# haoheliu/AudioLDM2

Hardware: AMD Instinct MI355X
Metric: audio_seconds_per_second (higher is better)
Workload: dtype f32 storage/accumulate; each product = 6 bf16 MFMA partial products of exact 3-part operand splits (fp32-grade); 1 GPU; audioldm2-full: batch 8 prompts/GPU x 1 GPU, 10.24 s @16 kHz, 200 DDIM steps, CFG 3.5, eta 1.0, n_candidates 1; one step = sample_log + VAE decode + HiFi-GAN + D2H of the waveform; synthetic conditioning, random-init weights, host-CPU RNG noise; global_batch=8, parallelism=prompt-sharded replicas x1, weight_broadcast_bytes=0

## Files before the change

audioldm2_amd/csrc/api.hip:

```cpp
#include "common.h"
#include <string.h>

namespace aldm {
static thread_local char g_err[512] = "";
void set_error(const char* fmt, ...) {
    va_list ap;
    va_start(ap, fmt);
    vsnprintf(g_err, sizeof(g_err), fmt, ap);
    va_end(ap);
}
}

extern "C" int aldm_version(void) { return 26; }
extern "C" const char* aldm_last_error(void) { return aldm::g_err; }
```

audioldm2_amd/csrc/norm.hip:

```cpp
#include <stdlib.h>
#include "igemm_epilogue.h"

namespace aldm {

constexpr int GN_ITERS = 16;
constexpr int GN_UNROLL = 8;

struct GnPart {
    float n, mean, m2;
};

__device__ __forceinline__ void gn_merge(double& n, double& mean, double& m2, double nb, double mb, double m2b) {
    if (nb <= 0.0) return;
    const double nt = n + nb;
    const double dlt = mb - mean;
    mean += dlt * (nb / nt);
    m2 += m2b + dlt * dlt * (n * nb / nt);
    n = nt;
}

template <bool FUSED>
__global__ __launch_bounds__(256) void gn_partial_kernel(const float* __restrict__ x1,
                                                         const float* __restrict__ x2, int P,
                                                         int C1, int C2, int G, int cols, int rows,
                                                         int chunk_px, float* __restrict__ ws, float eps,
                                                         const float* __restrict__ gamma,
                                                         const float* __restrict__ beta,
                                                         float* __restrict__ scale, float* __restrict__ shift, int gpb,
                                                         char* __restrict__ dst = nullptr, char* __restrict__ dst_raw = nullptr,
                                                         int parts = 3, int act = ALDM_ACT_NONE, int raw_parts = 3,
                                                         float f16_scale = 0.f) {
    const int C = C1 + C2;
    const int Cg4 = (C / G) >> 2;
    const int b = blockIdx.y;
    const int chunk = FUSED ? 0 : blockIdx.x;
    const int g_lo = FUSED ? blockIdx.x * gpb : 0;
    const int c4_lo = g_lo * Cg4, C4 = c4_lo + gpb * Cg4;
    const int p0 = chunk * chunk_px;
    const int p1 = min(P, p0 + chunk_px);
    const int tid = threadIdx.x;
    const int tx = tid % cols, ty = tid / cols;
    __shared__ GnPart ps[256];
    const int npass = (C4 - c4_lo + cols - 1) / cols;
    __shared__ double gacc[64][3];
    if (tid < 64) gacc[tid][0] = gacc[tid][1] = gacc[tid][2] = 0.0;
    __syncthreads();
    for (int cp = 0; cp < npass; ++cp) {
        const int c4 = c4_lo + cp * cols + tx;
        GnPart part = {0.f, 0.f, 0.f};
        if (ty < rows && c4 < C4 && p0 + ty < p1) {
            const int c = c4 << 2;
            const bool first = c < C1;
            const float* src = first ? x1 + (int64_t)b * P * C1 + c : x2 + (int64_t)b * P * C2 + (c - C1);
            const int pitch = first ? C1 : C2;
            float sa[GN_UNROLL], sq[GN_UNROLL];
#pragma unroll
            for (int u = 0; u < GN_UNROLL; ++u) sa[u] = sq[u] = 0.f;
            int p = p0 + ty;
            const f32x4 pv = *reinterpret_cast<const f32x4*>(src + (int64_t)p * pitch);
            const float pivot = fmaxf(fminf(pv[0], pv[1]), fminf(fmaxf(pv[0], pv[1]), pv[2]));
            int cnt = 0;
            for (; p + (GN_UNROLL - 1) * rows < p1; p += GN_UNROLL * rows) {
                f32x4 v[GN_UNROLL];
#pragma unroll
                for (int u = 0; u < GN_UNROLL; ++u)
                    v[u] = *reinterpret_cast<const f32x4*>(src + (int64_t)(p + u * rows) * pitch) - pivot;
#pragma unroll
                for (int u = 0; u < GN_UNROLL; ++u) {
// ... 87 lines not shown
            scale[(int64_t)b * C + c] = sc;
            shift[(int64_t)b * C + c] = sh;
            if (dst) {
                lsc[c - g_lo * Cg] = sc;
                lsh[c - g_lo * Cg] = sh;
            }
        }
        if (dst) {
            __syncthreads();
            const int c_lo = g_lo * Cg, sw = (gpb * Cg) >> 3;
            for (int i = tid; i < P * sw; i += 256) {
                const int p = i / sw;
                const int cl = (i - p * sw) << 3;
                const int c = c_lo + cl;
                const int64_t row = (int64_t)b * P + p;
                const float* src = c < C1 ? x1 + row * C1 + c : x2 + row * C2 + (c - C1);
                f32x4 v0 = *reinterpret_cast<const f32x4*>(src);
                f32x4 v1 = *reinterpret_cast<const f32x4*>(src + 4);
                const int64_t off = (row * (C >> 5) + (c >> 5)) * (64 * parts) + (c & 31) * 2;
                u32x2 p0[3], p1[3];
                if (dst_raw) {
                    const int64_t roff = (row * (C >> 5) + (c >> 5)) * (64 * raw_parts) + (c & 31) * 2;
                    split4_parts(v0, p0, raw_parts);
                    split4_parts(v1, p1, raw_parts);
#pragma unroll
                    for (int q = 0; q < 3; ++q)
                        if (q < raw_parts)
                            *reinterpret_cast<u32x4*>(dst_raw + roff + q * 64) = u32x4{p0[q][0], p0[q][1], p1[q][0], p1[q][1]};
                }
#pragma unroll
                for (int e = 0; e < 4; ++e) {
// ... 7 lines not shown
                        v1[e] = silu_fast(v1[e]);
                    }
                }
                split4_fmt(v0, p0, parts, f16_scale);
                split4_fmt(v1, p1, parts, f16_scale);
#pragma unroll
                for (int q = 0; q < 3; ++q)
                    if (q < parts) *reinterpret_cast<u32x4*>(dst + off + q * 64) = u32x4{p0[q][0], p0[q][1], p1[q][0], p1[q][1]};
            }
        }
    } else if (tid < G) {
        double* w = reinterpret_cast<double*>(ws) + ((int64_t)(b * gridDim.x + chunk) * G + tid) * 3;
        w[0] = gacc[tid][0];
        w[1] = gacc[tid][1];
        w[2] = gacc[tid][2];
    }
}

__global__ __launch_bounds__(256) void gn_finalize_kernel(const float* __restrict__ ws, int chunks,
                                                          int P, int C, int G, float eps,
                                                          const float* __restrict__ gamma,
                                                          const float* __restrict__ beta,
                                                          float* __restrict__ scale,
                                                          float* __restrict__ shift) {
    const int b = blockIdx.x;
    __shared__ float s_mean[64], s_rstd[64];
    __shared__ double s_part[256][3];
    const int Cg = C / G;
    const double* wsd = reinterpret_cast<const double*>(ws);
    const int LPG = 256 / G >= 1 ? 256 / G : 1;
    {
        const int g = threadIdx.x / LPG, l = threadIdx.x % LPG;
        double n = 0.0, mean = 0.0, m2 = 0.0;
        if (g < G) {
            for (int ch = l; ch < chunks; ch += LPG) {
                const double* w = wsd + ((int64_t)(b * chunks + ch) * G + g) * 3;
                gn_merge(n, mean, m2, w[0], w[1], w[2]);
            }
        }
        s_part[threadIdx.x][0] = n;
        s_part[threadIdx.x][1] = mean;
        s_part[threadIdx.x][2] = m2;
    }
    __syncthreads();
    if (threadIdx.x < G) {
        const int g = threadIdx.x;
        double n = 0.0, mean = 0.0, m2 = 0.0;
        for (int l = 0; l < LPG; ++l) gn_merge(n, mean, m2, s_part[g * LPG + l][0], s_part[g * LPG + l][1], s_part[g * LPG + l][2]);
        double var = n > 0.0 ? m2 / n : 0.0;
        if (var < 0.0) var = 0.0;
        s_mean[g] = (float)mean;
        s_rstd[g] = (float)(1.0 / sqrt(var + (double)eps));
    }
    __syncthreads();
    for (int c = threadIdx.x; c < C; c += blockDim.x) {
        const int g = c / Cg;
        const float ga = gamma ? gamma[c] : 1.f;
        const float be = beta ? beta[c] : 0.f;
        const float sc = s_rstd[g] * ga;
        scale[(int64_t)b * C + c] = sc;
        shift[(int64_t)b * C + c] = be - s_mean[g] * sc;
    }
}

constexpr int LN_MAXV = 8;

template <int MAXV, int R, bool RMS = false>
__global__ __launch_bounds__(256) void layernorm_kernel(const float* __restrict__ x,
                                                        float* __restrict__ y, int M, int C,
                                                        const float* __restrict__ gamma,
                                                        const float* __restrict__ beta, float eps,
                                                        void* __restrict__ y_split, int parts, float f16_scale) {
    const int lane = threadIdx.x & 63;
    const int row0 = (blockIdx.x * 4 + (threadIdx.x >> 6)) * R;
    if (row0 >= M) return;
    const int C4 = C >> 2;
// ... 152 lines not shown
        pl.cols = c4b < 256 ? c4b : 256;
        pl.rows = 256 / pl.cols;
        pl.chunk_px = P;
        pl.chunks = 1;
        pl.passes = (c4b + pl.cols - 1) / pl.cols;
    } else {
        pl.form = ALDM_GN_CHUNKED;
        gn_geometry(P, C, &pl.cols, &pl.rows, &pl.chunk_px, &pl.chunks);
        pl.passes = (C / 4 + pl.cols - 1) / pl.cols;
    }
    const int px = P < pl.chunk_px ? P : pl.chunk_px;
    pl.active = pl.cols * (pl.rows < px ? pl.rows : px);
    return pl;
}

}

using namespace aldm;

extern "C" int64_t aldm_gn_ws_floats(int B, int P, int C, int G) {
    int cols, rows, chunk_px, chunks;
    gn_geometry(P, C, &cols, &rows, &chunk_px, &chunks);
    return (int64_t)B * chunks * G * 6 + 2;
}

extern "C" int aldm_split_rows(const float* x1, const float* x2, int C1, int C2, int64_t rows, int P, const float* scale,
                               const float* shift, int act, void* dst, void* dst_raw, int parts, void* stream);
extern "C" int aldm_split_rows_f16(const float* x1, const float* x2, int C1, int C2, int64_t rows, int P, const float* scale,
                                   const float* shift, int act, float slope, void* dst, void* dst_raw, int raw_parts, float f16_scale,
                                   void* stream);
// ... 8 lines not shown
    ALDM_CHECK(!want_split || (C % 32 == 0 && C1 % 8 == 0 && C2 % 8 == 0),
               "aldm_groupnorm_plan: a split image needs (C1+C2) %% 32 == 0, C1 %% 8 == 0 (C1=%d C2=%d)", C1, C2);
    const GnPlan pl = groupnorm_plan(B, P, C, C1, G, want_split != 0);
    if (form) *form = pl.form;
    if (group_slices) *group_slices = pl.gs;
    if (groups_per_block) *groups_per_block = pl.gpb;
    if (chunks) *chunks = pl.chunks;
    if (chunk_px) *chunk_px = pl.chunk_px;
    if (cols) *cols = pl.cols;
    if (rows) *rows = pl.rows;
    if (passes) *passes = pl.passes;
    if (active_threads) *active_threads = pl.active;
    return 0;
}

static int groupnorm_launch(const float* x1, const float* x2, int B, int P, int C1, int C2, int G, float eps,
                            const float* gamma, const float* beta, float* scale, float* shift, float* ws, void* dst,
                            void* dst_raw, int parts, int act, void* stream, int raw_parts = 0, float f16_scale = 0.f) {
    if (raw_parts == 0) raw_parts = parts;
    if (!x2) C2 = 0;
    const int C = C1 + C2;
    ALDM_CHECK(x1 && scale && shift && ws, "aldm_groupnorm_stats: null pointer");
    ws = reinterpret_cast<float*>((reinterpret_cast<uintptr_t>(ws) + 7) & ~uintptr_t(7));
    ALDM_CHECK(G > 0 && G <= 64 && C % G == 0 && (C / G) % 4 == 0 && C1 % 4 == 0,
               "aldm_groupnorm_stats: need C%%G==0, (C/G)%%4==0, C1%%4==0 (C1=%d C2=%d G=%d)", C1, C2, G);
    const GnPlan pl = groupnorm_plan(B, P, C, C1, G, dst != nullptr);
    hipStream_t st = (hipStream_t)stream;
    if (pl.form == ALDM_GN_FUSED_SPLIT) {
        hipLaunchKernelGGL(gn_partial_kernel<true>, dim3(pl.gs, B), dim3(256), 0, st, x1, x2, P, C1, C2, G, pl.cols, pl.rows, P, ws,
                           eps, gamma, beta, scale, shift, pl.gpb, reinterpret_cast<char*>(dst),
                           reinterpret_cast<char*>(dst_raw), parts, act, raw_parts, f16_scale);
        ALDM_LAUNCH_CHECK("aldm_groupnorm_split");
        return 0;
    }
    if (pl.form == ALDM_GN_FUSED) {
        hipLaunchKernelGGL(gn_partial_kernel<true>, dim3(pl.gs, B), dim3(256), 0, st, x1, x2, P, C1, C2, G, pl.cols,
                           pl.rows, P, ws, eps, gamma, beta, scale, shift, pl.gpb, nullptr, nullptr, 3, ALDM_ACT_NONE);
    } else {
        hipLaunchKernelGGL(gn_partial_kernel<false>, dim3(pl.chunks, B), dim3(256), 0, st, x1, x2, P, C1, C2, G,
                           pl.cols, pl.rows, pl.chunk_px, ws, eps, gamma, beta, scale, shift, G);
        hipLaunchKernelGGL(gn_finalize_kernel, dim3(B), dim3(256), 0, st, ws, pl.chunks, P, C, G, eps, gamma,
                           beta, scale, shift);
    }
    ALDM_LAUNCH_CHECK("aldm_groupnorm_stats");
    if (dst) {
        if (f16_scale != 0.f)
            return aldm_split_rows_f16(x1, x2, C1, C2, (int64_t)B * P, P, scale, shift, act, 0.f, dst, dst_raw, raw_parts, f16_scale, stream);
        return aldm_split_rows(x1, x2, C1, C2, (int64_t)B * P, P, scale, shift, act, dst, dst_raw, parts, stream);
    }
    return 0;
}

extern "C" int aldm_groupnorm_stats(const float* x1, const float* x2, int B, int P, int C1, int C2,
                                    int G, float eps, const float* gamma, const float* beta,
                                    float* scale, float* shift, float* ws, void* stream) {
    return groupnorm_launch(x1, x2, B, P, C1, C2, G, eps, gamma, beta, scale, shift, ws, nullptr, nullptr, 3, ALDM_ACT_NONE,
                            stream);
}

extern "C" int aldm_groupnorm_split(const float* x1, const float* x2, int B, int P, int C1, int C2, int G, float eps,
                                    const float* gamma, const float* beta, int act, float* scale, float* shift, float* ws,
                                    void* dst, void* dst_raw, int parts, void* stream) {
    if (!x2) C2 = 0;
    ALDM_CHECK(dst != nullptr && (parts == 2 || parts == 3) && (C1 + C2) % 32 == 0 && C1 % 8 == 0 && C2 % 8 == 0,
               "aldm_groupnorm_split: need dst, parts 2|3, (C1+C2) %% 32 == 0, C1 %% 8 == 0 (C1=%d C2=%d)", C1, C2);
    ALDM_CHECK(act == ALDM_ACT_NONE || act == ALDM_ACT_SILU, "aldm_groupnorm_split: activation %d not supported", act);
    ALDM_CHECK(((reinterpret_cast<uintptr_t>(dst) | reinterpret_cast<uintptr_t>(dst_raw)) & 15) == 0,
               "aldm_groupnorm_split: split images must be 16-byte aligned");
    return groupnorm_launch(x1, x2, B, P, C1, C2, G, eps, gamma, beta, scale, shift, ws, dst, dst_raw, parts, act, stream);
}

extern "C" int aldm_groupnorm_split_f16(const float* x1, const float* x2, int B, int P, int C1, int C2, int G, float eps,
                                        const float* gamma, const float* beta, int act, float* scale, float* shift, float* ws,
                                        void* dst, void* dst_raw, int raw_parts, float f16_scale, void* stream) {
    if (!x2) C2 = 0;
    ALDM_CHECK(dst != nullptr && f16_scale > 0.0f && (raw_parts == 2 || raw_parts == 3) && (C1 + C2) % 32 == 0 && C1 % 8 == 0 && C2 % 8 == 0,
               "aldm_groupnorm_split_f16: need dst, f16_scale > 0, raw_parts 2|3, (C1+C2) %% 32 == 0, C1 %% 8 == 0 (C1=%d C2=%d)", C1, C2);
    ALDM_CHECK(act == ALDM_ACT_NONE || act == ALDM_ACT_SILU, "aldm_groupnorm_split_f16: activation %d not supported", act);
    ALDM_CHECK(((reinterpret_cast<uintptr_t>(dst) | reinterpret_cast<uintptr_t>(dst_raw)) & 15) == 0,
               "aldm_groupnorm_split_f16: split images must be 16-byte aligned");
    return groupnorm_launch(x1, x2, B, P, C1, C2, G, eps, gamma, beta, scale, shift, ws, dst, dst_raw, 2, act, stream, raw_parts, f16_scale);
}

static int layernorm_launch(const float* x, float* y, void* y_split, int parts, int M, int C, const float* gamma,
                            const float* beta, float eps, void* stream, const char* name, bool rms = false, float f16_scale = 0.f) {
    ALDM_CHECK(parts == 2 || parts == 3, "%s: parts must be 2 or 3", name);
    ALDM_CHECK(x && (y || y_split) && gamma && (beta || rms), "%s: null pointer", name);
    ALDM_CHECK(C % 4 == 0 && C <= 256 * LN_MAXV, "%s: C=%d must be a multiple of 4 and <= %d", name, C, 256 * LN_MAXV);
    ALDM_CHECK(y_split == nullptr || (C % 32 == 0 && (reinterpret_cast<uintptr_t>(y_split) & 15) == 0),
               "%s: a split-image output needs C %% 32 == 0 and 16-byte alignment", name);
    hipStream_t st = (hipStream_t)stream;
#define ALDM_LN(V_, R_)                                                                                             \
    do {                                                                                                            \
        if (rms)                                                                                                    \
            hipLaunchKernelGGL((layernorm_kernel<V_, R_, true>), dim3(cdiv(M, 4 * R_)), dim3(256), 0, st, x, y, M, C, \
                               gamma, beta, eps, y_split, parts, f16_scale);                                        \
// ... 80 lines not shown
```

audioldm2_amd/lib.py:

```python
from __future__ import annotations

import ctypes as C
import os

_HERE = os.path.dirname(os.path.abspath(__file__))
LIB_PATH = os.environ.get("ALDM_LIB_PATH") or os.path.join(_HERE, "libaldm_hip.so")
ABI_VERSION = 26

ACT_NONE, ACT_SILU, ACT_LRELU, ACT_TANH, ACT_LOGCLAMP, ACT_GELU, ACT_GELU_TANH = range(7)
B_PACKED, B_NT = 0, 1
EPI_PLAIN, EPI_GEGLU, EPI_QKV = 0, 1, 2
GN_CHUNKED, GN_FUSED, GN_FUSED_SPLIT = 0, 1, 2
FMT_BF16, FMT_F16 = 0, 1
EPI_FORM_GENERIC, EPI_FORM_PLAIN, EPI_FORM_ROWBIAS, EPI_FORM_RES = range(4)


class IgemmDesc(C.Structure):

    _fields_ = [
        ("x1", C.c_void_p), ("x2", C.c_void_p),
        ("C1", C.c_int32), ("C2", C.c_int32),
        ("pix1", C.c_int32), ("pix2", C.c_int32),
        ("B", C.c_int32), ("H", C.c_int32), ("W", C.c_int32),
        ("up_h", C.c_int32), ("up_w", C.c_int32),
# ... 76 lines not shown
    "aldm_igemm_mma": (C.c_int, [C.c_int]),
    "aldm_split_bytes": (C.c_int64, [C.c_int, C.c_int]),
    "aldm_pack_split_bf16": (C.c_int, [C.c_void_p, C.c_void_p, C.c_int, C.c_int, C.c_void_p]),
    "aldm_pack_weight": (C.c_int, [C.c_void_p, C.c_void_p, C.c_int, C.c_int, C.c_int, C.c_int,
                                   C.c_int, C.c_int, C.c_int, C.c_void_p]),
    "aldm_pack_kn": (C.c_int, [C.c_void_p, C.c_void_p, C.c_int, C.c_int, C.c_int, C.c_int,
                               C.c_int64, C.c_int64, C.c_void_p]),
    "aldm_groupnorm_stats": (C.c_int, [C.c_void_p, C.c_void_p, C.c_int, C.c_int, C.c_int, C.c_int,
                                       C.c_int, C.c_float, C.c_void_p, C.c_void_p, C.c_void_p,
                                       C.c_void_p, C.c_void_p, C.c_void_p]),
    "aldm_gn_ws_floats": (C.c_int64, [C.c_int, C.c_int, C.c_int, C.c_int]),
    "aldm_groupnorm_plan": (C.c_int, [C.c_int] * 6 + [C.POINTER(C.c_int)] * 9),
    "aldm_groupnorm_split": (C.c_int, [C.c_void_p, C.c_void_p, C.c_int, C.c_int, C.c_int, C.c_int, C.c_int, C.c_float,
                                       C.c_void_p, C.c_void_p, C.c_int, C.c_void_p, C.c_void_p, C.c_void_p, C.c_void_p,
                                       C.c_void_p, C.c_int, C.c_void_p]),
    "aldm_layernorm": (C.c_int, [C.c_void_p, C.c_void_p, C.c_int, C.c_int, C.c_void_p, C.c_void_p,
                                 C.c_float, C.c_void_p]),
    "aldm_attention_mma": (C.c_int, [C.c_int]),
    "aldm_attention_sched": (C.c_int, [C.c_int]),
    "aldm_attention_query_tiles": (C.c_int, [C.c_int, C.c_int, C.c_int]),
    "aldm_attention_d32_presplit_f16": (C.c_int, [C.c_void_p, C.c_void_p, C.c_void_p, C.c_void_p, C.c_void_p, C.c_int, C.c_float,
                                                  C.c_int, C.c_int, C.c_int, C.c_int, C.c_int, C.c_int, C.c_float, C.c_float,
                                                  C.c_float, C.c_float, C.c_void_p]),
    "aldm_attention_d32_presplit": (C.c_int, [C.c_void_p, C.c_void_p, C.c_void_p, C.c_void_p, C.c_void_p, C.c_int, C.c_int,
                                              C.c_int, C.c_int, C.c_int, C.c_int, C.c_int, C.c_float, C.c_void_p]),
    "aldm_vt_regroup": (C.c_int, [C.c_void_p, C.c_void_p, C.c_int, C.c_int, C.c_int, C.c_int, C.c_void_p]),
    "aldm_attention_d32": (C.c_int, [C.c_void_p, C.c_void_p, C.c_void_p, C.c_void_p, C.c_int,
                                     C.c_int, C.c_int, C.c_int, C.c_int, C.c_int, C.c_int, C.c_int,
                                     C.c_void_p, C.c_float, C.c_void_p]),
    "aldm_rel_attention": (C.c_int, [C.c_void_p, C.c_void_p, C.c_void_p, C.c_void_p, C.c_int, C.c_int, C.c_int, C.c_int,
# ... 169 lines not shown
```

audioldm2_amd/ops.py:

```python
from __future__ import annotations

import ctypes as C
import json
import os
from dataclasses import dataclass
from typing import List, Optional, Sequence, Tuple

import torch

from . import lib as _l
from .lib import (ACT_GELU, ACT_GELU_TANH, ACT_LOGCLAMP, ACT_LRELU, ACT_NONE, ACT_SILU, ACT_TANH, B_NT, B_PACKED,
                  IgemmDesc)


def _stream() -> int:
    return torch.cuda.current_stream().cuda_stream


def _p(t: Optional[torch.Tensor]):
    return None if t is None else t.data_ptr()


def _chk(t: torch.Tensor, name: str):
    if not (t.is_cuda and t.dtype == torch.float32 and t.is_contiguous()):
# ... 821 lines not shown

GN_FORMS = ("chunked", "fused", "fused_split")


def groupnorm_plan(B: int, P: int, C1: int, C2: int = 0, groups: int = 32, want_split: bool = False) -> dict:
    import ctypes
    out = [ctypes.c_int() for _ in range(9)]
    _l.check(_l.load().aldm_groupnorm_plan(B, P, C1, C2, groups, 1 if want_split else 0, *[ctypes.byref(o) for o in out]),
             "groupnorm_plan")
    keys = ("form", "group_slices", "groups_per_block", "chunks", "chunk_px", "cols", "rows", "passes", "active_threads")
    plan = {k: o.value for k, o in zip(keys, out)}
    plan["form"] = GN_FORMS[plan["form"]]
    return plan


def gn_split(x: torch.Tensor, gamma: torch.Tensor, beta: torch.Tensor, *, groups: int = 32, eps: float = 1e-5,
             x2: Optional[torch.Tensor] = None, act: int = ACT_NONE, want_raw: bool = False):
    _chk(x, "gn_split.x")
    B = x.shape[0]
    C1 = x.shape[-1]
    P = x.numel() // (B * C1)
    C2 = 0
    if x2 is not None:
        _chk(x2, "gn_split.x2")
        assert x2.shape[:-1] == x.shape[:-1]
        C2 = x2.shape[-1]
    Cc = C1 + C2
    lib = _l.load()
    ws = torch.empty(lib.aldm_gn_ws_floats(B, P, Cc, groups), device=x.device, dtype=torch.float32)
    ss = torch.empty((2, B, Cc), device=x.device, dtype=torch.float32)
    shape = (*x.shape[:-1], Cc)
    raw = SplitT.empty(shape, x.device) if want_raw else None
    if f16_mode():
        dst = SplitT.empty(shape, x.device, f16_scale=_norm_f16_scale(gamma, beta, (Cc // groups) * P))
        _l.check(lib.aldm_groupnorm_split_f16(x.data_ptr(), _p(x2), B, P, C1, C2, groups, eps, gamma.data_ptr(), beta.data_ptr(), act,
                                              ss[0].data_ptr(), ss[1].data_ptr(), ws.data_ptr(), dst.data_ptr(),
                                              None if raw is None else raw.data_ptr(), 3, dst.scale, _stream()), "groupnorm_split_f16")
        return (dst, raw) if want_raw else dst
    dst = SplitT.empty(shape, x.device)
    _l.check(lib.aldm_groupnorm_split(x.data_ptr(), _p(x2), B, P, C1, C2, groups, eps, gamma.data_ptr(), beta.data_ptr(), act,
                                      ss[0].data_ptr(), ss[1].data_ptr(), ws.data_ptr(), dst.data_ptr(),
                                      None if raw is None else raw.data_ptr(), dst.parts, _stream()), "groupnorm_split")
    return (dst, raw) if want_raw else dst


def layernorm(x: torch.Tensor, gamma: torch.Tensor, beta: torch.Tensor, eps: float = 1e-5,
              split_out: Optional[str] = None):
    _chk(x, "ln.x")
    Cc = x.shape[-1]
    M = x.numel() // Cc
    y = None if split_out == "only" else torch.empty_like(x)
    if not split_out:
        _l.check(_l.load().aldm_layernorm(x.data_ptr(), y.data_ptr(), M, Cc, gamma.data_ptr(),
                                          beta.data_ptr(), eps, _stream()), "layernorm")
        return y
    if f16_mode():
        so = SplitT.empty(x.shape, x.device, f16_scale=_norm_f16_scale(gamma, beta, Cc))
        so.rn = _row_norm_bound(gamma, beta, Cc)
# ... 859 lines not shown
```

audioldm2_amd/unet.py:

```python
from __future__ import annotations

from typing import List, Optional

import torch
import torch.nn as nn

import os

from . import ops
from .ops import ACT_NONE, ACT_SILU

PRESPLIT_ATTENTION = os.environ.get("ALDM_ATTN_PRESPLIT", "1") != "0" and "ALDM_ATTN_MMA" not in os.environ


class ResBlock(nn.Module):

    def __init__(self, channels, emb_channels, dropout, out_channels=None):
        super().__init__()
        self.channels = channels
        self.out_channels = out_channels or channels
        self.in_layers = nn.Sequential(nn.GroupNorm(32, channels), nn.SiLU(),
                                       nn.Conv2d(channels, self.out_channels, 3, padding=1))
        self.emb_layers = nn.Sequential(nn.SiLU(), nn.Linear(emb_channels, self.out_channels))
        self.out_layers = nn.Sequential(nn.GroupNorm(32, self.out_channels), nn.SiLU(), nn.Dropout(p=dropout),
# ... 20 lines not shown
        return self._pk

    def run(self, x, e, x2=None):
        pk = self._prepare()
        c2 = 0 if x2 is None else x2.shape[-1]
        if ops.use_dma() and self.channels % 32 == 0 and x.shape[-1] % 8 == 0 and c2 % 8 == 0:
            if pk["skip"] is None:
                assert x2 is None
                a1, skip = ops.gn_split(x, *pk["gn1"], groups=32, eps=1e-5, act=ACT_SILU), x
            else:
                a1, araw = ops.gn_split(x, *pk["gn1"], groups=32, eps=1e-5, x2=x2, act=ACT_SILU, want_raw=True)
                skip = ops.conv(araw, pk["skip"])
            h = ops.conv(a1, pk["conv1"], pad=(1, 1), rowbias=e)
            a2 = ops.gn_split(h, *pk["gn2"], groups=32, eps=1e-5, act=ACT_SILU)
            return ops.conv(a2, pk["conv2"], pad=(1, 1), res=skip)
        sc, sh = ops.gn_stats(x, *pk["gn1"], groups=32, eps=1e-5, x2=x2)
        h = ops.conv(x, pk["conv1"], x2=x2, pad=(1, 1), pre=(sc, sh), pre_act=ACT_SILU, rowbias=e)
        sc2, sh2 = ops.gn_stats(h, *pk["gn2"], groups=32, eps=1e-5)
        if pk["skip"] is None:
            assert x2 is None
            skip = x
        else:
            skip = ops.conv(x, pk["skip"], x2=x2)
        return ops.conv(h, pk["conv2"], pad=(1, 1), pre=(sc2, sh2), pre_act=ACT_SILU, res=skip)


class Downsample(nn.Module):

    def __init__(self, channels, use_conv=True, dims=2, out_channels=None, padding=1):
        super().__init__()
# ... 422 lines not shown
        else:
            dup = lambda t: t.repeat(2, *([1] * (t.dim() - 1)))
            emb_half, emb = emb, _EmbSlices(dup(emb_rows))
            for bi, module in enumerate(self.input_blocks):
                if bi < div[0]:
                    h = module.run(h, emb_half, context_list, mask_list)
                elif bi == div[0]:
                    h = module.run(h, emb_half, context_list, mask_list, hi=div[1])
                    h = module.run(dup(h), emb, context_list, mask_list, lo=div[1])
                else:
                    h = module.run(h, emb, context_list, mask_list)
                hs.append(h)
        h = self.middle_block.run(h, emb, context_list, mask_list)
        for module in self.output_blocks:
            skip = hs.pop()
            if skip.shape[0] != h.shape[0]:
                skip = dup(skip)
            h = module.run(h, emb, context_list, mask_list, x2=skip)
        sc, sh = ops.gn_stats(h, *pk["gn"], groups=32, eps=1e-5)
        out = ops.conv(h, pk["out"], pad=(1, 1), pre=(sc, sh), pre_act=ACT_SILU)
        return ops.nhwc_to_nchw(out)
```

include/aldm_hip.h:

```cpp
#ifndef ALDM_HIP_H
#define ALDM_HIP_H

#include <stdint.h>

#ifdef __cplusplus
extern "C" {
#endif

int aldm_version(void);
const char* aldm_last_error(void);

enum {
    ALDM_ACT_NONE = 0,
    ALDM_ACT_SILU = 1,
    ALDM_ACT_LRELU = 2,
    ALDM_ACT_TANH = 3,
    ALDM_ACT_LOGCLAMP = 4,
    ALDM_ACT_GELU = 5,
    ALDM_ACT_GELU_TANH = 6
};

enum { ALDM_EPI_PLAIN = 0, ALDM_EPI_GEGLU = 1, ALDM_EPI_QKV = 2 };

enum {
// ... 97 lines not shown

int aldm_groupnorm_stats(const float* x1, const float* x2, int B, int P, int C1, int C2,
                         int G, float eps, const float* gamma, const float* beta,
                         float* scale, float* shift, float* ws, void* stream);
int64_t aldm_gn_ws_floats(int B, int P, int C, int G);
enum { ALDM_GN_CHUNKED = 0, ALDM_GN_FUSED = 1, ALDM_GN_FUSED_SPLIT = 2 };
int aldm_groupnorm_plan(int B, int P, int C1, int C2, int G, int want_split, int* form, int* group_slices,
                        int* groups_per_block, int* chunks, int* chunk_px, int* cols, int* rows, int* passes,
                        int* active_threads);
int aldm_groupnorm_split(const float* x1, const float* x2, int B, int P, int C1, int C2, int G, float eps,
                         const float* gamma, const float* beta, int act, float* scale, float* shift, float* ws,
                         void* dst, void* dst_raw, int parts, void* stream);
int aldm_groupnorm_split_f16(const float* x1, const float* x2, int B, int P, int C1, int C2, int G, float eps,
                             const float* gamma, const float* beta, int act, float* scale, float* shift, float* ws,
                             void* dst, void* dst_raw, int raw_parts, float f16_scale, void* stream);
int aldm_layernorm(const float* x, float* y, int M, int C, const float* gamma,
                   const float* beta, float eps, void* stream);
int aldm_layernorm_split(const float* x, float* y, void* y_split, int M, int C, const float* gamma,
                         const float* beta, float eps, int parts, void* stream);
int aldm_layernorm_split_f16(const float* x, float* y, void* y_split, int M, int C, const float* gamma,
                             const float* beta, float eps, float f16_scale, void* stream);

int aldm_attention_d32(const float* q, const float* k, const float* v, float* out,
                       int B, int heads, int Lq, int Lk, int ldq, int ldk, int ldv, int ldo,
                       const float* mask, float scale, void* stream);
int aldm_attention_d32_split(const float* q, const float* k, const float* v, float* out, void* out_split,
                             int parts, int B, int heads, int Lq, int Lk, int ldq, int ldk, int ldv, int ldo,
                             const float* mask, float scale, void* stream);
int aldm_attention_d32_presplit(const float* q, const void* k_split, const void* vt_split, float* out, void* out_split,
                                int parts, int B, int heads, int Lq, int Lk, int ldq, int ldo, float scale, void* stream);
// ... 131 lines not shown
```

Baseline: 19.67 audio-s/s.

## Fold GroupNorm finalize into split-apply kernel and broadcast skip inputs in place

Adds a gn_apply_split kernel that recomputes per-sample group statistics from the chunked partials inside each block and then normalizes, activates and splits the concatenated input. This removes the separate finalize launch and its global round trip for scale/shift. It also lets the second (skip) input hold fewer samples than the first and index it by b % B2, so the UNet decoder no longer duplicates skip tensors for the CFG batch. The cost is redundant per-block finalize work and a smaller apply grid (divided by 4 by default); both features can be switched off via environment variables.

Measured after the change: 19.75 audio-s/s (median of 6 runs). No clear change (+0.4%).

```diff
diff --git a/audioldm2_amd/csrc/api.hip b/audioldm2_amd/csrc/api.hip
--- a/audioldm2_amd/csrc/api.hip
+++ b/audioldm2_amd/csrc/api.hip
@@ -11,5 +11,5 @@
 }
 }
 
-extern "C" int aldm_version(void) { return 26; }
+extern "C" int aldm_version(void) { return 27; }
 extern "C" const char* aldm_last_error(void) { return aldm::g_err; }
diff --git a/audioldm2_amd/csrc/norm.hip b/audioldm2_amd/csrc/norm.hip
--- a/audioldm2_amd/csrc/norm.hip
+++ b/audioldm2_amd/csrc/norm.hip
@@ -1,4 +1,6 @@
 #include <stdlib.h>
+#include <algorithm>
+#include <atomic>
 #include "igemm_epilogue.h"
 
 namespace aldm {
@@ -27,12 +29,14 @@
                                                          const float* __restrict__ gamma,
                                                          const float* __restrict__ beta,
                                                          float* __restrict__ scale, float* __restrict__ shift, int gpb,
+                                                         int B2,
                                                          char* __restrict__ dst = nullptr, char* __restrict__ dst_raw = nullptr,
                                                          int parts = 3, int act = ALDM_ACT_NONE, int raw_parts = 3,
                                                          float f16_scale = 0.f) {
     const int C = C1 + C2;
     const int Cg4 = (C / G) >> 2;
     const int b = blockIdx.y;
+    const int b2 = b % B2;
     const int chunk = FUSED ? 0 : blockIdx.x;
     const int g_lo = FUSED ? blockIdx.x * gpb : 0;
     const int c4_lo = g_lo * Cg4, C4 = c4_lo + gpb * Cg4;
@@ -51,7 +55,7 @@
         if (ty < rows && c4 < C4 && p0 + ty < p1) {
             const int c = c4 << 2;
             const bool first = c < C1;
-            const float* src = first ? x1 + (int64_t)b * P * C1 + c : x2 + (int64_t)b * P * C2 + (c - C1);
+            const float* src = first ? x1 + (int64_t)b * P * C1 + c : x2 + (int64_t)b2 * P * C2 + (c - C1);
             const int pitch = first ? C1 : C2;
             float sa[GN_UNROLL], sq[GN_UNROLL];
 #pragma unroll
@@ -169,7 +173,7 @@
                 const int cl = (i - p * sw) << 3;
                 const int c = c_lo + cl;
                 const int64_t row = (int64_t)b * P + p;
-                const float* src = c < C1 ? x1 + row * C1 + c : x2 + row * C2 + (c - C1);
+                const float* src = c < C1 ? x1 + row * C1 + c : x2 + ((int64_t)b2 * P + p) * C2 + (c - C1);
                 f32x4 v0 = *reinterpret_cast<const f32x4*>(src);
                 f32x4 v1 = *reinterpret_cast<const f32x4*>(src + 4);
                 const int64_t off = (row * (C >> 5) + (c >> 5)) * (64 * parts) + (c & 31) * 2;
@@ -207,6 +211,59 @@
         w[0] = gacc[tid][0];
         w[1] = gacc[tid][1];
         w[2] = gacc[tid][2];
+    }
+}
+
+__device__ __forceinline__ void gn_finalize_sample(const float* __restrict__ ws, int chunks, int b, int C, int G, float eps,
+                                                   const float* __restrict__ gamma, const float* __restrict__ beta,
+                                                   double (*s_part)[3], float* s_mean, float* s_rstd, float* sc_out,
+                                                   float* sh_out) {
+    const int Cg = C / G;
+    const double* wsd = reinterpret_cast<const double*>(ws);
+    const int LPG = 256 / G >= 1 ? 256 / G : 1;
+    {
+        const int g = threadIdx.x / LPG, l = threadIdx.x % LPG;
+        double n = 0.0, mean = 0.0, m2 = 0.0;
+        if (g < G) {
+            for (int ch0 = l; ch0 < chunks; ch0 += 4 * LPG) {
+                double w[4][3];
+#pragma unroll
+                for (int u = 0; u < 4; ++u) {
+                    const int ch = ch0 + u * LPG;
+                    w[u][0] = w[u][1] = w[u][2] = 0.0;
+                    if (ch < chunks) {
+                        const double* wp = wsd + ((int64_t)(b * chunks + ch) * G + g) * 3;
+                        w[u][0] = wp[0];
+                        w[u][1] = wp[1];
+                        w[u][2] = wp[2];
+                    }
+                }
+#pragma unroll
+                for (int u = 0; u < 4; ++u) gn_merge(n, mean, m2, w[u][0], w[u][1], w[u][2]);
+            }
+        }
+        s_part[threadIdx.x][0] = n;
+        s_part[threadIdx.x][1] = mean;
+        s_part[threadIdx.x][2] = m2;
+    }
+    __syncthreads();
+    if (threadIdx.x < G) {
+        const int g = threadIdx.x;
+        double n = 0.0, mean = 0.0, m2 = 0.0;
+        for (int l = 0; l < LPG; ++l) gn_merge(n, mean, m2, s_part[g * LPG + l][0], s_part[g * LPG + l][1], s_part[g * LPG + l][2]);
+        double var = n > 0.0 ? m2 / n : 0.0;
+        if (var < 0.0) var = 0.0;
+        s_mean[g] = (float)mean;
+        s_rstd[g] = (float)(1.0 / sqrt(var + (double)eps));
+    }
+    __syncthreads();
+    for (int c = threadIdx.x; c < C; c += blockDim.x) {
+        const int g = c / Cg;
+        const float ga = gamma ? gamma[c] : 1.f;
+        const float be = beta ? beta[c] : 0.f;
+        const float sc = s_rstd[g] * ga;
+        sc_out[c] = sc;
+        sh_out[c] = be - s_mean[g] * sc;
     }
 }
 
@@ -219,40 +276,91 @@
     const int b = blockIdx.x;
     __shared__ float s_mean[64], s_rstd[64];
     __shared__ double s_part[256][3];
-    const int Cg = C / G;
-    const double* wsd = reinterpret_cast<const double*>(ws);
-    const int LPG = 256 / G >= 1 ? 256 / G : 1;
-    {
-        const int g = threadIdx.x / LPG, l = threadIdx.x % LPG;
-        double n = 0.0, mean = 0.0, m2 = 0.0;
-        if (g < G) {
-            for (int ch = l; ch < chunks; ch += LPG) {
-                const double* w = wsd + ((int64_t)(b * chunks + ch) * G + g) * 3;
-                gn_merge(n, mean, m2, w[0], w[1], w[2]);
-            }
-        }
-        s_part[threadIdx.x][0] = n;
-        s_part[threadIdx.x][1] = mean;
-        s_part[threadIdx.x][2] = m2;
-    }
+    gn_finalize_sample(ws, chunks, b, C, G, eps, gamma, beta, s_part, s_mean, s_rstd, scale + (int64_t)b * C, shift + (int64_t)b * C);
+}
+
+constexpr int GN_FOLD_SCRATCH = 256 * 3 * 8 + 2 * 64 * 4;
+constexpr int GN_FOLD_MAX_C = 4096;
+
+template <int ACT>
+__global__ __launch_bounds__(256) void gn_apply_split_kernel(const float* __restrict__ x1, const float* __restrict__ x2, int B2,
+                                                             int P, int C1, int C2, int G, const float* __restrict__ ws,
+                                                             int chunks, float eps, const float* __restrict__ gamma,
+                                                             const float* __restrict__ beta, float* __restrict__ scale,
+                                                             float* __restrict__ shift, char* __restrict__ dst,
+                                                             char* __restrict__ dst_raw, int parts, int raw_parts,
+                                                             float f16_scale) {
+    extern __shared__ __attribute__((aligned(16))) char gn_fold_smem[];
+    double (*s_part)[3] = reinterpret_cast<double (*)[3]>(gn_fold_smem);
+    float* s_mean = reinterpret_cast<float*>(gn_fold_smem + 256 * 3 * 8);
+    float* s_rstd = s_mean + 64;
+    float* lsc = s_rstd + 64;
+    const int C = C1 + C2;
+    const int C8 = C >> 3;
+    float* lsh = lsc + C;
+    const int b = blockIdx.y;
+    const int items = P * C8;
+    const int step = gridDim.x * 256;
+    const float* xb1 = x1 + (int64_t)b * P * C1;
+    const float* xb2 = x2 + (int64_t)(b % B2) * P * C2;
+    int i = blockIdx.x * 256 + threadIdx.x;
+    f32x4 n0 = {0.f, 0.f, 0.f, 0.f}, n1 = n0;
+    if (i < items) {
+        const int p = i / C8;
+        const int c = (i - p * C8) << 3;
+        const float* src = c < C1 ? xb1 + (int64_t)p * C1 + c : xb2 + (int64_t)p * C2 + (c - C1);
+        n0 = *reinterpret_cast<const f32x4*>(src);
+        n1 = *reinterpret_cast<const f32x4*>(src + 4);
+    }
+    gn_finalize_sample(ws, chunks, b, C, G, eps, gamma, beta, s_part, s_mean, s_rstd, lsc, lsh);
     __syncthreads();
-    if (threadIdx.x < G) {
-        const int g = threadIdx.x;
-        double n = 0.0, mean = 0.0, m2 = 0.0;
-        for (int l = 0; l < LPG; ++l) gn_merge(n, mean, m2, s_part[g * LPG + l][0], s_part[g * LPG + l][1], s_part[g * LPG + l][2]);
-        double var = n > 0.0 ? m2 / n : 0.0;
-        if (var < 0.0) var = 0.0;
-        s_mean[g] = (float)mean;
-        s_rstd[g] = (float)(1.0 / sqrt(var + (double)eps));
-    }
-    __syncthreads();
-    for (int c = threadIdx.x; c < C; c += blockDim.x) {
-        const int g = c / Cg;
-        const float ga = gamma ? gamma[c] : 1.f;
-        const float be = beta ? beta[c] : 0.f;
-        const float sc = s_rstd[g] * ga;
-        scale[(int64_t)b * C + c] = sc;
-        shift[(int64_t)b * C + c] = be - s_mean[g] * sc;
+    if (blockIdx.x == 0) {
+        for (int c = threadIdx.x; c < C; c += 256) {
+            scale[(int64_t)b * C + c] = lsc[c];
+            shift[(int64_t)b * C + c] = lsh[c];
+        }
+    }
+    for (; i < items; i += step) {
+        const int p = i / C8;
+        const int c = (i - p * C8) << 3;
+        f32x4 v0 = n0, v1 = n1;
+        if (i + step < items) {
+            const int pn = (i + step) / C8;
+            const int cn = ((i + step) - pn * C8) << 3;
+            const float* src = cn < C1 ? xb1 + (int64_t)pn * C1 + cn : xb2 + (int64_t)pn * C2 + (cn - C1);
+            n0 = *reinterpret_cast<const f32x4*>(src);
+            n1 = *reinterpret_cast<const f32x4*>(src + 4);
+        }
+        const int64_t row = (int64_t)b * P + p;
+        const int64_t off = (row * (C >> 5) + (c >> 5)) * (64 * parts) + (c & 31) * 2;
+        u32x2 p0[3], p1[3];
+        if (dst_raw) {
+            const int64_t roff = (row * (C >> 5) + (c >> 5)) * (64 * raw_parts) + (c & 31) * 2;
+            split4_parts(v0, p0, raw_parts);
+            split4_parts(v1, p1, raw_parts);
+#pragma unroll
+            for (int q = 0; q < 3; ++q)
+                if (q < raw_parts) *reinterpret_cast<u32x4*>(dst_raw + roff + q * 64) = u32x4{p0[q][0], p0[q][1], p1[q][0], p1[q][1]};
+        }
+        const f32x4 s0 = *reinterpret_cast<const f32x4*>(lsc + c), s1 = *reinterpret_cast<const f32x4*>(lsc + c + 4);
+        const f32x4 h0 = *reinterpret_cast<const f32x4*>(lsh + c), h1 = *reinterpret_cast<const f32x4*>(lsh + c + 4);
+#pragma unroll
+        for (int e = 0; e < 4; ++e) {
+            v0[e] = __builtin_fmaf(v0[e], s0[e], h0[e]);
+            v1[e] = __builtin_fmaf(v1[e], s1[e], h1[e]);
+        }
+        if constexpr (ACT == ALDM_ACT_SILU) {
+#pragma unroll
+            for (int e = 0; e < 4; ++e) {
+                v0[e] = silu_fast(v0[e]);
+                v1[e] = silu_fast(v1[e]);
+            }
+        }
+        split4_fmt(v0, p0, parts, f16_scale);
+        split4_fmt(v1, p1, parts, f16_scale);
+#pragma unroll
+        for (int q = 0; q < 3; ++q)
+            if (q < parts) *reinterpret_cast<u32x4*>(dst + off + q * 64) = u32x4{p0[q][0], p0[q][1], p1[q][0], p1[q][1]};
     }
 }
 
@@ -435,6 +543,46 @@
     return pl;
 }
 
+static std::atomic<int> g_gn_fold{-1};
+static int gn_fold_on() {
+    static const int env_on = [] {
+        const char* e = getenv("ALDM_GN_FOLD");
+        return (e && e[0] == '0' && e[1] == 0) ? 0 : 1;
+    }();
+    const int v = g_gn_fold.load(std::memory_order_relaxed);
+    return v < 0 ? env_on : v;
+}
+
+constexpr int GN_FOLD_GRID_CAP = 256 * 16;
+
+struct GnFold {
+    int launches;
+    int nblk;
+};
+
+static GnFold gn_fold_plan(const GnPlan& pl, int B, int P, int C, bool want_split) {
+    GnFold f;
+    f.nblk = 0;
+    if (pl.form == ALDM_GN_FUSED_SPLIT) {
+        f.launches = 1;
+        return f;
+    }
+    f.launches = (pl.form == ALDM_GN_CHUNKED ? 2 : 1) + (want_split ? 1 : 0);
+    const int64_t items = (int64_t)P * (C >> 3);
+    if (pl.form != ALDM_GN_CHUNKED || !want_split || !gn_fold_on() || C > GN_FOLD_MAX_C || items >= ((int64_t)1 << 30) || B > 65535)
+        return f;
+    static const int div = [] {
+        const char* e = getenv("ALDM_GN_FOLD_DIV");
+        const int v = e ? atoi(e) : 0;
+        return v >= 1 ? v : 4;
+    }();
+    const int per_sample = GN_FOLD_GRID_CAP / B >= 1 ? GN_FOLD_GRID_CAP / B : 1;
+    const int64_t full = std::min<int64_t>((items + 255) / 256, per_sample);
+    f.nblk = (int)std::max<int64_t>(full / div, 1);
+    f.launches = 2;
+    return f;
+}
+
 }
 
 using namespace aldm;
@@ -473,31 +621,72 @@
     return 0;
 }
 
-static int groupnorm_launch(const float* x1, const float* x2, int B, int P, int C1, int C2, int G, float eps,
+extern "C" int aldm_groupnorm_fold_plan(int B, int P, int C1, int C2, int G, int want_split, int* launches, int* nblk) {
+    const int C = C1 + C2;
+    ALDM_CHECK(B > 0 && P > 0 && C1 > 0 && C2 >= 0, "aldm_groupnorm_fold_plan: bad shape (B=%d P=%d C1=%d C2=%d)", B, P, C1, C2);
+    ALDM_CHECK(G > 0 && G <= 64 && C % G == 0 && (C / G) % 4 == 0 && C1 % 4 == 0,
+               "aldm_groupnorm_fold_plan: need C%%G==0, (C/G)%%4==0, C1%%4==0 (C1=%d C2=%d G=%d)", C1, C2, G);
+    ALDM_CHECK(!want_split || (C % 32 == 0 && C1 % 8 == 0 && C2 % 8 == 0),
+               "aldm_groupnorm_fold_plan: a split image needs (C1+C2) %% 32 == 0, C1 %% 8 == 0 (C1=%d C2=%d)", C1, C2);
+    const GnFold f = gn_fold_plan(groupnorm_plan(B, P, C, C1, G, want_split != 0), B, P, C, want_split != 0);
+    if (launches) *launches = f.launches;
+    if (nblk) *nblk = f.nblk;
+    return 0;
+}
+
+extern "C" int aldm_gn_fold_finalize(int on) {
+    const int prev = gn_fold_on();
+    g_gn_fold.store(on == 0 || on == 1 ? on : -1, std::memory_order_relaxed);
+    return prev;
+}
+
+static int groupnorm_launch(const float* x1, const float* x2, int B2, int B, int P, int C1, int C2, int G, float eps,
                             const float* gamma, const float* beta, float* scale, float* shift, float* ws, void* dst,
                             void* dst_raw, int parts, int act, void* stream, int raw_parts = 0, float f16_scale = 0.f) {
     if (raw_parts == 0) raw_parts = parts;
-    if (!x2) C2 = 0;
+    if (!x2) {
+        C2 = 0;
+        B2 = B;
+    }
     const int C = C1 + C2;
     ALDM_CHECK(x1 && scale && shift && ws, "aldm_groupnorm_stats: null pointer");
+    ALDM_CHECK(B > 0 && B2 > 0 && B % B2 == 0, "aldm_groupnorm_stats: x2 must hold a divisor of B samples (B=%d B2=%d)", B, B2);
     ws = reinterpret_cast<float*>((reinterpret_cast<uintptr_t>(ws) + 7) & ~uintptr_t(7));
     ALDM_CHECK(G > 0 && G <= 64 && C % G == 0 && (C / G) % 4 == 0 && C1 % 4 == 0,
                "aldm_groupnorm_stats: need C%%G==0, (C/G)%%4==0, C1%%4==0 (C1=%d C2=%d G=%d)", C1, C2, G);
     const GnPlan pl = groupnorm_plan(B, P, C, C1, G, dst != nullptr);
+    const GnFold fold = gn_fold_plan(pl, B, P, C, dst != nullptr);
     hipStream_t st = (hipStream_t)stream;
     if (pl.form == ALDM_GN_FUSED_SPLIT) {
         hipLaunchKernelGGL(gn_partial_kernel<true>, dim3(pl.gs, B), dim3(256), 0, st, x1, x2, P, C1, C2, G, pl.cols, pl.rows, P, ws,
-                           eps, gamma, beta, scale, shift, pl.gpb, reinterpret_cast<char*>(dst),
+                           eps, gamma, beta, scale, shift, pl.gpb, B2, reinterpret_cast<char*>(dst),
                            reinterpret_cast<char*>(dst_raw), parts, act, raw_parts, f16_scale);
         ALDM_LAUNCH_CHECK("aldm_groupnorm_split");
         return 0;
     }
+    ALDM_CHECK(B2 == B || dst == nullptr || fold.nblk > 0,
+               "aldm_groupnorm_split: x2 with fewer samples than x1 (B=%d B2=%d) needs the fused-split or the folded form", B, B2);
     if (pl.form == ALDM_GN_FUSED) {
         hipLaunchKernelGGL(gn_partial_kernel<true>, dim3(pl.gs, B), dim3(256), 0, st, x1, x2, P, C1, C2, G, pl.cols,
-                           pl.rows, P, ws, eps, gamma, beta, scale, shift, pl.gpb, nullptr, nullptr, 3, ALDM_ACT_NONE);
+                           pl.rows, P, ws, eps, gamma, beta, scale, shift, pl.gpb, B2, nullptr, nullptr, 3, ALDM_ACT_NONE);
     } else {
         hipLaunchKernelGGL(gn_partial_kernel<false>, dim3(pl.chunks, B), dim3(256), 0, st, x1, x2, P, C1, C2, G,
-                           pl.cols, pl.rows, pl.chunk_px, ws, eps, gamma, beta, scale, shift, G);
+                           pl.cols, pl.rows, pl.chunk_px, ws, eps, gamma, beta, scale, shift, G, B2);
+        if (fold.nblk > 0) {
+            ALDM_CHECK(((reinterpret_cast<uintptr_t>(x1) | reinterpret_cast<uintptr_t>(x2)) & 15) == 0,
+                       "aldm_groupnorm_split: operands must be 16-byte aligned");
+            const size_t lds = GN_FOLD_SCRATCH + (size_t)C * 8;
+            const dim3 grid(fold.nblk, B);
+#define ALDM_GN_APPLY(A_)                                                                                                  \
+    hipLaunchKernelGGL((gn_apply_split_kernel<A_>), grid, dim3(256), lds, st, x1, x2, B2, P, C1, C2, G, ws, pl.chunks, eps, \
+                       gamma, beta, scale, shift, reinterpret_cast<char*>(dst), reinterpret_cast<char*>(dst_raw), parts,   \
+                       raw_parts, f16_scale)
+            if (act == ALDM_ACT_SILU) ALDM_GN_APPLY(ALDM_ACT_SILU);
+            else ALDM_GN_APPLY(ALDM_ACT_NONE);
+#undef ALDM_GN_APPLY
+            ALDM_LAUNCH_CHECK("aldm_groupnorm_split");
+            return 0;
+        }
         hipLaunchKernelGGL(gn_finalize_kernel, dim3(B), dim3(256), 0, st, ws, pl.chunks, P, C, G, eps, gamma,
                            beta, scale, shift);
     }
@@ -513,32 +702,46 @@
 extern "C" int aldm_groupnorm_stats(const float* x1, const float* x2, int B, int P, int C1, int C2,
                                     int G, float eps, const float* gamma, const float* beta,
                                     float* scale, float* shift, float* ws, void* stream) {
-    return groupnorm_launch(x1, x2, B, P, C1, C2, G, eps, gamma, beta, scale, shift, ws, nullptr, nullptr, 3, ALDM_ACT_NONE,
+    return groupnorm_launch(x1, x2, B, B, P, C1, C2, G, eps, gamma, beta, scale, shift, ws, nullptr, nullptr, 3, ALDM_ACT_NONE,
                             stream);
 }
 
-extern "C" int aldm_groupnorm_split(const float* x1, const float* x2, int B, int P, int C1, int C2, int G, float eps,
-                                    const float* gamma, const float* beta, int act, float* scale, float* shift, float* ws,
-                                    void* dst, void* dst_raw, int parts, void* stream) {
+extern "C" int aldm_groupnorm_split_x2b(const float* x1, const float* x2, int B2, int B, int P, int C1, int C2, int G, float eps,
+                                        const float* gamma, const float* beta, int act, float* scale, float* shift, float* ws,
+                                        void* dst, void* dst_raw, int parts, void* stream) {
     if (!x2) C2 = 0;
     ALDM_CHECK(dst != nullptr && (parts == 2 || parts == 3) && (C1 + C2) % 32 == 0 && C1 % 8 == 0 && C2 % 8 == 0,
                "aldm_groupnorm_split: need dst, parts 2|3, (C1+C2) %% 32 == 0, C1 %% 8 == 0 (C1=%d C2=%d)", C1, C2);
     ALDM_CHECK(act == ALDM_ACT_NONE || act == ALDM_ACT_SILU, "aldm_groupnorm_split: activation %d not supported", act);
     ALDM_CHECK(((reinterpret_cast<uintptr_t>(dst) | reinterpret_cast<uintptr_t>(dst_raw)) & 15) == 0,
                "aldm_groupnorm_split: split images must be 16-byte aligned");
-    return groupnorm_launch(x1, x2, B, P, C1, C2, G, eps, gamma, beta, scale, shift, ws, dst, dst_raw, parts, act, stream);
-}
-
-extern "C" int aldm_groupnorm_split_f16(const float* x1, const float* x2, int B, int P, int C1, int C2, int G, float eps,
-                                        const float* gamma, const float* beta, int act, float* scale, float* shift, float* ws,
-                                        void* dst, void* dst_raw, int raw_parts, float f16_scale, void* stream) {
+    return groupnorm_launch(x1, x2, B2, B, P, C1, C2, G, eps, gamma, beta, scale, shift, ws, dst, dst_raw, parts, act, stream);
+}
+
+extern "C" int aldm_groupnorm_split(const float* x1, const float* x2, int B, int P, int C1, int C2, int G, float eps,
+                                    const float* gamma, const float* beta, int act, float* scale, float* shift, float* ws,
+                                    void* dst, void* dst_raw, int parts, void* stream) {
+    return aldm_groupnorm_split_x2b(x1, x2, B, B, P, C1, C2, G, eps, gamma, beta, act, scale, shift, ws, dst, dst_raw, parts, stream);
+}
+
+extern "C" int aldm_groupnorm_split_x2b_f16(const float* x1, const float* x2, int B2, int B, int P, int C1, int C2, int G, float eps,
+                                            const float* gamma, const float* beta, int act, float* scale, float* shift, float* ws,
+                                            void* dst, void* dst_raw, int raw_parts, float f16_scale, void* stream) {
     if (!x2) C2 = 0;
     ALDM_CHECK(dst != nullptr && f16_scale > 0.0f && (raw_parts == 2 || raw_parts == 3) && (C1 + C2) % 32 == 0 && C1 % 8 == 0 && C2 % 8 == 0,
                "aldm_groupnorm_split_f16: need dst, f16_scale > 0, raw_parts 2|3, (C1+C2) %% 32 == 0, C1 %% 8 == 0 (C1=%d C2=%d)", C1, C2);
     ALDM_CHECK(act == ALDM_ACT_NONE || act == ALDM_ACT_SILU, "aldm_groupnorm_split_f16: activation %d not supported", act);
     ALDM_CHECK(((reinterpret_cast<uintptr_t>(dst) | reinterpret_cast<uintptr_t>(dst_raw)) & 15) == 0,
                "aldm_groupnorm_split_f16: split images must be 16-byte aligned");
-    return groupnorm_launch(x1, x2, B, P, C1, C2, G, eps, gamma, beta, scale, shift, ws, dst, dst_raw, 2, act, stream, raw_parts, f16_scale);
+    return groupnorm_launch(x1, x2, B2, B, P, C1, C2, G, eps, gamma, beta, scale, shift, ws, dst, dst_raw, 2, act, stream, raw_parts,
+                            f16_scale);
+}
+
+extern "C" int aldm_groupnorm_split_f16(const float* x1, const float* x2, int B, int P, int C1, int C2, int G, float eps,
+                                        const float* gamma, const float* beta, int act, float* scale, float* shift, float* ws,
+                                        void* dst, void* dst_raw, int raw_parts, float f16_scale, void* stream) {
+    return aldm_groupnorm_split_x2b_f16(x1, x2, B, B, P, C1, C2, G, eps, gamma, beta, act, scale, shift, ws, dst, dst_raw, raw_parts,
+                                        f16_scale, stream);
 }
 
 static int layernorm_launch(const float* x, float* y, void* y_split, int parts, int M, int C, const float* gamma,
diff --git a/audioldm2_amd/lib.py b/audioldm2_amd/lib.py
--- a/audioldm2_amd/lib.py
+++ b/audioldm2_amd/lib.py
@@ -5,7 +5,7 @@
 
 _HERE = os.path.dirname(os.path.abspath(__file__))
 LIB_PATH = os.environ.get("ALDM_LIB_PATH") or os.path.join(_HERE, "libaldm_hip.so")
-ABI_VERSION = 26
+ABI_VERSION = 27
 
 ACT_NONE, ACT_SILU, ACT_LRELU, ACT_TANH, ACT_LOGCLAMP, ACT_GELU, ACT_GELU_TANH = range(7)
 B_PACKED, B_NT = 0, 1
@@ -114,6 +114,14 @@
     "aldm_groupnorm_split": (C.c_int, [C.c_void_p, C.c_void_p, C.c_int, C.c_int, C.c_int, C.c_int, C.c_int, C.c_float,
                                        C.c_void_p, C.c_void_p, C.c_int, C.c_void_p, C.c_void_p, C.c_void_p, C.c_void_p,
                                        C.c_void_p, C.c_int, C.c_void_p]),
+    "aldm_groupnorm_split_x2b": (C.c_int, [C.c_void_p, C.c_void_p, C.c_int, C.c_int, C.c_int, C.c_int, C.c_int, C.c_int, C.c_float,
+                                           C.c_void_p, C.c_void_p, C.c_int, C.c_void_p, C.c_void_p, C.c_void_p, C.c_void_p,
+                                           C.c_void_p, C.c_int, C.c_void_p]),
+    "aldm_groupnorm_split_x2b_f16": (C.c_int, [C.c_void_p, C.c_void_p, C.c_int, C.c_int, C.c_int, C.c_int, C.c_int, C.c_int,
+                                               C.c_float, C.c_void_p, C.c_void_p, C.c_int, C.c_void_p, C.c_void_p, C.c_void_p,
+                                               C.c_void_p, C.c_void_p, C.c_int, C.c_float, C.c_void_p]),
+    "aldm_gn_fold_finalize": (C.c_int, [C.c_int]),
+    "aldm_groupnorm_fold_plan": (C.c_int, [C.c_int] * 6 + [C.POINTER(C.c_int)] * 2),
     "aldm_layernorm": (C.c_int, [C.c_void_p, C.c_void_p, C.c_int, C.c_int, C.c_void_p, C.c_void_p,
                                  C.c_float, C.c_void_p]),
     "aldm_attention_mma": (C.c_int, [C.c_int]),
diff --git a/audioldm2_amd/ops.py b/audioldm2_amd/ops.py
--- a/audioldm2_amd/ops.py
+++ b/audioldm2_amd/ops.py
@@ -859,34 +859,68 @@
     return plan
 
 
+def gn_fold_finalize(on: int = -1) -> int:
+    return _l.load().aldm_gn_fold_finalize(on)
+
+
+def groupnorm_fold_plan(B: int, P: int, C1: int, C2: int = 0, groups: int = 32, want_split: bool = True) -> dict:
+    import ctypes
+    launches, nblk = ctypes.c_int(), ctypes.c_int()
+    _l.check(_l.load().aldm_groupnorm_fold_plan(B, P, C1, C2, groups, 1 if want_split else 0, ctypes.byref(launches),
+                                                ctypes.byref(nblk)), "groupnorm_fold_plan")
+    return {"launches": launches.value, "nblk": nblk.value}
+
+
+GN_SKIP_IN_PLACE = os.environ.get("ALDM_GN_SKIP_IN_PLACE", "1") != "0"
+
+
+def gn_skip_in_place(on=None):
+    global GN_SKIP_IN_PLACE
+    prev = GN_SKIP_IN_PLACE
+    if on is not None:
+        GN_SKIP_IN_PLACE = bool(on)
+    return prev
+
+
 def gn_split(x: torch.Tensor, gamma: torch.Tensor, beta: torch.Tensor, *, groups: int = 32, eps: float = 1e-5,
-             x2: Optional[torch.Tensor] = None, act: int = ACT_NONE, want_raw: bool = False):
+             x2: Optional[torch.Tensor] = None, act: int = ACT_NONE, want_raw: bool = False, want_stats: bool = False):
     _chk(x, "gn_split.x")
     B = x.shape[0]
     C1 = x.shape[-1]
     P = x.numel() // (B * C1)
     C2 = 0
+    B2 = B
+    lib = _l.load()
     if x2 is not None:
         _chk(x2, "gn_split.x2")
-        assert x2.shape[:-1] == x.shape[:-1]
+        B2 = x2.shape[0]
+        assert x2.shape[1:-1] == x.shape[1:-1] and B2 > 0 and B % B2 == 0
         C2 = x2.shape[-1]
+        if B2 != B and groupnorm_plan(B, P, C1, C2, groups, True)["form"] != "fused_split" \
+                and groupnorm_fold_plan(B, P, C1, C2, groups)["nblk"] == 0:
+            x2 = x2.repeat(B // B2, *([1] * (x2.dim() - 1)))
+            B2 = B
     Cc = C1 + C2
-    lib = _l.load()
     ws = torch.empty(lib.aldm_gn_ws_floats(B, P, Cc, groups), device=x.device, dtype=torch.float32)
     ss = torch.empty((2, B, Cc), device=x.device, dtype=torch.float32)
     shape = (*x.shape[:-1], Cc)
     raw = SplitT.empty(shape, x.device) if want_raw else None
     if f16_mode():
         dst = SplitT.empty(shape, x.device, f16_scale=_norm_f16_scale(gamma, beta, (Cc // groups) * P))
-        _l.check(lib.aldm_groupnorm_split_f16(x.data_ptr(), _p(x2), B, P, C1, C2, groups, eps, gamma.data_ptr(), beta.data_ptr(), act,
-                                              ss[0].data_ptr(), ss[1].data_ptr(), ws.data_ptr(), dst.data_ptr(),
-                                              None if raw is None else raw.data_ptr(), 3, dst.scale, _stream()), "groupnorm_split_f16")
-        return (dst, raw) if want_raw else dst
+        _l.check(lib.aldm_groupnorm_split_x2b_f16(x.data_ptr(), _p(x2), B2, B, P, C1, C2, groups, eps, gamma.data_ptr(),
+                                                  beta.data_ptr(), act, ss[0].data_ptr(), ss[1].data_ptr(), ws.data_ptr(),
+                                                  dst.data_ptr(), None if raw is None else raw.data_ptr(), 3, dst.scale, _stream()),
+                 "groupnorm_split_f16")
+        out = (dst, raw) if want_raw else (dst,)
+        out = out + ((ss[0], ss[1]),) if want_stats else out
+        return out if len(out) > 1 else dst
     dst = SplitT.empty(shape, x.device)
-    _l.check(lib.aldm_groupnorm_split(x.data_ptr(), _p(x2), B, P, C1, C2, groups, eps, gamma.data_ptr(), beta.data_ptr(), act,
-                                      ss[0].data_ptr(), ss[1].data_ptr(), ws.data_ptr(), dst.data_ptr(),
-                                      None if raw is None else raw.data_ptr(), dst.parts, _stream()), "groupnorm_split")
-    return (dst, raw) if want_raw else dst
+    _l.check(lib.aldm_groupnorm_split_x2b(x.data_ptr(), _p(x2), B2, B, P, C1, C2, groups, eps, gamma.data_ptr(), beta.data_ptr(), act,
+                                          ss[0].data_ptr(), ss[1].data_ptr(), ws.data_ptr(), dst.data_ptr(),
+                                          None if raw is None else raw.data_ptr(), dst.parts, _stream()), "groupnorm_split")
+    out = (dst, raw) if want_raw else (dst,)
+    out = out + ((ss[0], ss[1]),) if want_stats else out
+    return out if len(out) > 1 else dst
 
 
 def layernorm(x: torch.Tensor, gamma: torch.Tensor, beta: torch.Tensor, eps: float = 1e-5,
diff --git a/audioldm2_amd/unet.py b/audioldm2_amd/unet.py
--- a/audioldm2_amd/unet.py
+++ b/audioldm2_amd/unet.py
@@ -58,6 +58,8 @@
             h = ops.conv(a1, pk["conv1"], pad=(1, 1), rowbias=e)
             a2 = ops.gn_split(h, *pk["gn2"], groups=32, eps=1e-5, act=ACT_SILU)
             return ops.conv(a2, pk["conv2"], pad=(1, 1), res=skip)
+        if x2 is not None and x2.shape[0] != x.shape[0]:
+            x2 = x2.repeat(x.shape[0] // x2.shape[0], *([1] * (x2.dim() - 1)))
         sc, sh = ops.gn_stats(x, *pk["gn1"], groups=32, eps=1e-5, x2=x2)
         h = ops.conv(x, pk["conv1"], x2=x2, pad=(1, 1), pre=(sc, sh), pre_act=ACT_SILU, rowbias=e)
         sc2, sh2 = ops.gn_stats(h, *pk["gn2"], groups=32, eps=1e-5)
@@ -510,7 +512,7 @@
         h = self.middle_block.run(h, emb, context_list, mask_list)
         for module in self.output_blocks:
             skip = hs.pop()
-            if skip.shape[0] != h.shape[0]:
+            if skip.shape[0] != h.shape[0] and not ops.GN_SKIP_IN_PLACE:
                 skip = dup(skip)
             h = module.run(h, emb, context_list, mask_list, x2=skip)
         sc, sh = ops.gn_stats(h, *pk["gn"], groups=32, eps=1e-5)
diff --git a/include/aldm_hip.h b/include/aldm_hip.h
--- a/include/aldm_hip.h
+++ b/include/aldm_hip.h
@@ -135,6 +135,14 @@
 int aldm_groupnorm_split_f16(const float* x1, const float* x2, int B, int P, int C1, int C2, int G, float eps,
                              const float* gamma, const float* beta, int act, float* scale, float* shift, float* ws,
                              void* dst, void* dst_raw, int raw_parts, float f16_scale, void* stream);
+int aldm_groupnorm_split_x2b(const float* x1, const float* x2, int B2, int B, int P, int C1, int C2, int G, float eps,
+                             const float* gamma, const float* beta, int act, float* scale, float* shift, float* ws,
+                             void* dst, void* dst_raw, int parts, void* stream);
+int aldm_groupnorm_split_x2b_f16(const float* x1, const float* x2, int B2, int B, int P, int C1, int C2, int G, float eps,
+                                 const float* gamma, const float* beta, int act, float* scale, float* shift, float* ws,
+                                 void* dst, void* dst_raw, int raw_parts, float f16_scale, void* stream);
+int aldm_gn_fold_finalize(int on);
+int aldm_groupnorm_fold_plan(int B, int P, int C1, int C2, int G, int want_split, int* launches, int* nblk);
 int aldm_layernorm(const float* x, float* y, int M, int C, const float* gamma,
                    const float* beta, float eps, void* stream);
 int aldm_layernorm_split(const float* x, float* y, void* y_split, int M, int C, const float* gamma,
```
